# timdestan/go-raytracer

Measured on AMD Instinct MI355X. Metric: Mrays/s (primary+shadow+reflect) at 4K depth=6; 1/2/4/8-GPU scaling, higher is better.
Workload: dtype f64; 1 GPU; c3: cylinder + cube + sphere (cone substitute) over a reflective plane, 4 lights, 3840x2160, depth 6; width=3840, height=2160, depth=6, lights=4, objects=4, parallelism=rows1-interleaved, frames_in_flight=2, schedule=auto, kernel=specialised, accel=bvh+cull

## Files before the change

go-raytracer_amd/csrc/rt_kernel.hip:

```cpp
#pragma clang fp contract(off)

#include <hip/hip_runtime.h>

#include <dlfcn.h>
#include <errno.h>
#include <fcntl.h>
#include <hip/hiprtc.h>
#include <sys/syscall.h>
#include <sys/wait.h>
#include <unistd.h>

#include <algorithm>
#include <atomic>
#include <chrono>
#include <condition_variable>
#include <cstdlib>
#include <functional>
#include <thread>
#include <cmath>
#include <array>
#include <cstdio>
#include <utility>
#include <cstring>
#include <limits>
// ... 466 lines not shown
  uint64_t* gboard = nullptr;
  uint64_t* gring = nullptr;
  uint64_t* gctl = nullptr;
  size_t gslots = 0;
  int gframes = 0;
  unsigned int* est = nullptr;
  size_t est_cap = 0;
  unsigned long long* est_stats = nullptr;
  std::vector<uint32_t> tile_cost;
  double order_ms = 0;
  std::map<std::array<int, 5>, unsigned int*> orders;
  bool specialize = false;
  int accel = RT_ACCEL_BVH | RT_ACCEL_CULL;
  hipFunction_t spec_fn = nullptr;
  std::map<int, hipFunction_t> spec_alt;
  SpecKey spec_key;
  double spec_ms = 0;
  bool spec_async = false;
  bool spec_fallback = false;
  bool spec_pending = false;
  bool spec_failed = false;
  std::string spec_err;
  bool last_spec = false;
};

namespace {

struct DeviceGuard {
  int prev = -1;
  explicit DeviceGuard(int dev) {
    if (hipGetDevice(&prev) != hipSuccess) prev = -1;
    if (prev != dev) (void)hipSetDevice(dev);
  }
  ~DeviceGuard() {
    if (prev >= 0) (void)hipSetDevice(prev);
  }
};

void free_scene(DevScene& s) {
  (void)hipFree(s.blob);
  (void)hipFree(s.accel);
  s = DevScene();
}

void clear_orders(rt_context* c) {
  for (auto& kv : c->orders) (void)hipFree(kv.second);
// ... 1443 lines not shown
  {
    const int top = n / topd;
    const int tail = taild > 0 ? std::min(n - top, n / taild) : 0;
    std::vector<char> cls(n, 1);
    for (int i = 0; i < top; i++) cls[ord[i]] = 0;
    for (int i = n - tail; i < n; i++) cls[ord[i]] = 2;
    int k = top;
    for (int v = 0; v < n; v++)
      if (cls[v] == 1) ord[k++] = (uint32_t)v;
    for (int v = 0; v < n; v++)
      if (cls[v] == 2) ord[k++] = (uint32_t)v;
  }
  unsigned int* d = nullptr;
  HIP_TRY(hipMalloc((void**)&d, (size_t)n * sizeof(unsigned int)));
  if (hipMemcpy(d, ord.data(), (size_t)n * sizeof(unsigned int), hipMemcpyHostToDevice) != hipSuccess) {
    (void)hipFree(d);
    return fail(RT_E_DEVICE, "tile order upload failed");
  }
  c->orders[key] = d;
  *out = d;
  return RT_OK;
}

static int launch(rt_context* c, int y0, int y1, int trow0, int stride, int ntrows, void* d_rgba, void* stream,
                  bool est) {
  const DevScene& s = c->sc;
  DeviceGuard guard(c->device);
  hipStream_t st = (hipStream_t)stream;
  if (c->spec_pending && !est) (void)spec_prepare(c);
  const bool lds = scene_in_lds(s);
  const int vm_off = lds ? s.blob_bytes : 0;
  const int stack_off = vm_off + ((lds && s.num_programs) ? WG * MAT * (int)sizeof(double) : 0);
  const int cnt_off = stack_off + (s.use_bvh ? WAVES_PER_WG * BVH_STACK * 12 : 0);
  const int qmask_off = cnt_off + CNT_BYTES;
  const int jump_off = qmask_off + 16;
  const int board_off = jump_off + 20 * 4 * (int)sizeof(uint64_t);
  const uint64_t launch_pixels = (uint64_t)s.width * (uint64_t)(stride > 0 ? ntrows * TILE : y1 - y0);
  const int sch =
      est ? (int)SCH_SERIAL : pick_schedule(c->sched, s, launch_pixels, c->cus, c->inflight, c->spec_fn != nullptr);
  const int share_m = (c->spec_fn && !est) ? pick_share(c->share_mode, s, launch_pixels, c->cus, c->inflight) : 0;
  hipFunction_t spec = nullptr;
  if (!est) {
    int rc = spec_for(c, sch, share_m, &spec);
    if (rc != RT_OK) return rc;
  }
  static const bool spec_extra = rt_getenv("RT_SPEC_EXTRA_FLAGS") != nullptr;
  const bool use_stream = !lds && !s.use_bvh && !s.has_csg && (spec_extra || !(spec && !(c->accel & RT_ACCEL_CULL)));
  const bool quads = sch == SCH_QUADS || (sch == SCH_PAIRS && !spec);
  const void* kfn = k_kernels[kernel_index(lds, s.use_bvh, s.has_csg, quads, s.ext_code)];
  const bool share = spec && share_m == RT_SHARE_GROUP;
  const int stream_off = board_off + (share ? BOARD_BYTES : 0);
  const int frames_off = stream_off + (use_stream ? WAVES_PER_WG * SCH * (GEO * (int)sizeof(double) + (int)sizeof(int)) : 0);
  int shmem = frames_off;
  auto occupancy = [&](int bytes) {
    int n = 0;
    if (spec) {
      if (hipModuleOccupancyMaxActiveBlocksPerMultiprocessor(&n, spec, WG, bytes) != hipSuccess) n = 0;
    } else if (hipOccupancyMaxActiveBlocksPerMultiprocessor(&n, kfn, WG, bytes) != hipSuccess) {
      n = 0;
    }
    return n;
  };
  const void* plan_fn = spec ? (const void*)spec : kfn;
  const int frames = std::max(1, s.depth - 1);
  LaunchPlan& pl = c->plan;
  const bool plan_hit = pl.fn == plan_fn && pl.shmem_fixed == shmem && pl.frames == frames;
  int per_cu = plan_hit ? pl.per_cu : occupancy(shmem);
  if (per_cu <= 0) per_cu = 1;
  const int level_bytes = WAVES_PER_WG * CORE * 64 * (int)sizeof(double);
  const int ext_bytes = WAVES_PER_WG * EXT_ROWS * 64 * (int)sizeof(double);
  int lds_levels = plan_hit ? pl.lds_levels : 0, lds_full = plan_hit ? pl.lds_full : 0;
  if (!plan_hit && c->lds_per_cu > 0 && c->lds_per_block > 0) {
    const int avail = std::min(c->lds_per_block, c->lds_per_cu / std::min(per_cu, 8)) - shmem;
    if (const char* e = rt_getenv("RT_LDS_FULL")) lds_full = std::max(0, std::min(frames, atoi(e)));
    while (lds_full > 0 && lds_full * (ext_bytes + level_bytes) > avail) lds_full--;
    lds_levels = std::max(lds_full, std::min(frames, (avail - lds_full * ext_bytes) / level_bytes));
    if (const char* e = rt_getenv("RT_LDS_LEVELS")) lds_levels = std::max(lds_full, std::min(lds_levels, atoi(e)));
    while (lds_levels > 0 && occupancy(shmem + lds_levels * level_bytes + lds_full * ext_bytes) < per_cu) {
      lds_levels--;
      lds_full = std::min(lds_full, lds_levels);
    }
  }
  if (!plan_hit) pl = LaunchPlan{plan_fn, shmem, frames, per_cu, lds_levels, lds_full};
  const int ext_off = shmem + lds_levels * level_bytes;
  shmem = ext_off + lds_full * ext_bytes;
  static const bool dbg = rt_getenv("RT_DEBUG_LAUNCH") != nullptr;
  if (dbg)
    fprintf(stderr, "[launch] blocks/CU %d, LDS/block %d B (fixed %d, frame cores %d levels, full frames %d levels), frames %d\n",
            per_cu, shmem, frames_off, lds_levels, lds_full, frames);
  const int grid = c->cus * std::min(per_cu, 8);
  c->last_waves = grid * WAVES_PER_WG;
  c->launches++;
  if (grid * WAVES_PER_WG > c->stack_waves) return fail(RT_E_INVALID, "frame stack smaller than the grid");
  if (spec && share_m == RT_SHARE_DEVICE) {
    const size_t need = (size_t)c->stack_waves * 64 * frames;
    if (need != c->gslots || frames != c->gframes) {
      (void)hipFree(c->gboard);
      c->gboard = nullptr;
      c->gslots = 0;
      if (hipExtMallocWithFlags((void**)&c->gboard, need * GS_REC * sizeof(uint64_t), hipDeviceMallocUncached) !=
          hipSuccess)
        return fail(RT_E_NOMEM, "device-wide work-sharing slots");
      if (!c->gring && hipExtMallocWithFlags((void**)&c->gring, (size_t)GS_RING * sizeof(uint64_t),
                                             hipDeviceMallocUncached) != hipSuccess)
        return fail(RT_E_NOMEM, "device-wide work-sharing ring");
      if (!c->gctl && hipExtMallocWithFlags((void**)&c->gctl, GS_CTL_U64 * sizeof(uint64_t), hipDeviceMallocUncached) !=
                          hipSuccess)
        return fail(RT_E_NOMEM, "device-wide work-sharing control");
      HIP_TRY(hipMemsetAsync(c->gboard, 0, need * GS_REC * sizeof(uint64_t), st));
      HIP_TRY(hipMemsetAsync(c->gring, 0, (size_t)GS_RING * sizeof(uint64_t), st));
      HIP_TRY(hipMemsetAsync(c->gctl, 0, GS_CTL_U64 * sizeof(uint64_t), st));
      c->gslots = need;
      c->gframes = frames;
    }
  }
  Params P;
  std::memset(&P, 0, sizeof P);
  P.lds_frames_off = frames_off;
  P.lds_levels = lds_levels;
  P.lds_full = lds_full;
  P.stream_off = stream_off;
  P.lds_ext_off = ext_off;
  P.qmask_off = qmask_off;
  P.jump_off = jump_off;
  P.board_off = board_off;
  P.gboard = c->gboard;
  P.gring = c->gring;
  P.gctl = c->gctl;
  P.gslots = c->gslots;
  P.gset = c->qset;
  P.off_geo = s.off_geo;
  P.off_shade = s.off_shade;
  P.off_mats = s.off_mats;
  P.off_lights = s.off_lights;
  P.off_kind = s.off_kind;
  P.off_objmat = s.off_objmat;
  P.off_pref = s.off_prefb;
  P.off_csg = s.off_csg;
  P.off_code = s.off_code;
  P.off_consts = s.off_consts;
  P.off_entry = s.off_entry;
  P.lds_vm_off = vm_off;
  P.vm_global = c->vm_global;
  P.blob_bytes = s.blob_bytes;
  P.jump = c->jump;
  P.queue = c->queue + c->qset * QSET_ALLOC;
  P.queue_next = c->queue + (1 - c->qset) * QSET_ALLOC;
  P.stats = est ? c->est_stats : c->stats;
// ... 112 lines not shown
  c->order_ms = std::chrono::duration<double, std::milli>(std::chrono::steady_clock::now() - t0).count();
  c->timed = false;
  return RT_OK;
}

int rt_set_work_sharing(rt_context* c, int enable) {
  if (!c) return fail(RT_E_INVALID, "rt_set_work_sharing: NULL context");
  if (enable < 0 || enable > RT_SHARE_AUTO) return fail(RT_E_INVALID, "rt_set_work_sharing: unknown mode");
  c->share_mode = enable;
  return c->has_scene ? spec_prepare(c) : RT_OK;
}

int rt_set_tile_order(rt_context* c, int enable) {
  if (!c) return fail(RT_E_INVALID, "rt_set_tile_order: NULL context");
  c->order_on = enable != 0;
  if (!c->has_scene) return RT_OK;
  if (!c->order_on) {
    clear_orders(c);
    return RT_OK;
  }
  return c->tile_cost.empty() ? estimate_costs(c) : RT_OK;
}

int rt_tile_order_info(rt_context* c, int* active, double* estimate_ms) {
  if (!c || !active || !estimate_ms) return fail(RT_E_INVALID, "rt_tile_order_info: NULL argument");
  *active = c->tile_cost.empty() ? 0 : 1;
  *estimate_ms = c->order_ms;
  return RT_OK;
}

int rt_render_rows_async(rt_context* c, int y0, int y1, void* d_rgba, void* stream) {
  if (!c || !c->has_scene) return fail(RT_E_INVALID, "rt_render_rows_async: no scene set");
  if (!d_rgba) return fail(RT_E_INVALID, "rt_render_rows_async: NULL output");
  if (y0 < 0 || y1 > c->sc.height || y1 <= y0) return fail(RT_E_INVALID, "rt_render_rows_async: bad row range");
  return launch(c, y0, y1, 0, 0, 0, d_rgba, stream, false);
}

int rt_render_tile_rows_async(rt_context* c, int trow0, int trow_stride, int ntrows, void* d_rgba, void* stream) {
  if (!c || !c->has_scene) return fail(RT_E_INVALID, "rt_render_tile_rows_async: no scene set");
  if (!d_rgba) return fail(RT_E_INVALID, "rt_render_tile_rows_async: NULL output");
  if (trow0 < 0 || trow_stride <= 0 || ntrows <= 0) return fail(RT_E_INVALID, "rt_render_tile_rows_async: bad tile rows");
  return launch(c, 0, c->sc.height, trow0, trow_stride, ntrows, d_rgba, stream, false);
}


int rt_read_stats(rt_context* c, void* stream, int reset, rt_stats* out) {
// ... 182 lines not shown
```

go-raytracer_amd/csrc/rt_render.h:

```cpp
#pragma once
#pragma clang fp contract(off)

#ifndef __HIPCC_RTC__
#include <hip/hip_runtime.h>
#endif

#include "rt_abi.h"
#include "rt_device.h"

#ifndef RT_SHADE_NUM
#define RT_SHADE_NUM 3
#endif
#ifndef RT_SHADE_DEN
#define RT_SHADE_DEN 4
#endif
#ifndef RT_DIV_SKIP
#define RT_DIV_SKIP 0
#endif
#ifndef RT_PIX_BATCH
#define RT_PIX_BATCH 1
#endif
#ifndef RT_PAIRS
#define RT_PAIRS 0
#endif
// ... 121 lines not shown
  int trow0, trow_stride;
  unsigned int total_slots;
  int frames;
  const float* bvh_nodes;
  const double* bvh_geo;
  const int* planes;
  int nplanes, bvh_stack_off;
  double bvh_lo[3], bvh_hi[3];
  const int* runs;
  int nruns;
  const double* arec;
  const double* urec;
  int cnt_off;
  int kind_mask;
  int board_off;
  uint64_t* gboard;
  uint64_t* gring;
  uint64_t* gctl;
  int gset;
  unsigned long long gslots;
  const unsigned int* order;
  unsigned int* est_out;
  int est_pts;
};
enum { CNT_TRACED = 0, CNT_SHADED = 1, CNT_SURFERR = 2, NUNIT = 3, CNT_KIND_OFF = 128,
       CNT_BYTES = CNT_KIND_OFF + RT_NUM_KINDS * WG * 8 };
enum { PREF = 8 };
enum { BN = 16, BVH_STACK = 64 };

struct Ray {
  d3 o, d;
};

template <typename MP>
__device__ __forceinline__ d3 to_obj_o(MP m, d3 o) {
  return mk(m[0] * o.x + m[1] * o.y + m[2] * o.z + m[3], m[4] * o.x + m[5] * o.y + m[6] * o.z + m[7],
            m[8] * o.x + m[9] * o.y + m[10] * o.z + m[11]);
}
template <typename MP>
__device__ __forceinline__ d3 to_obj_d(MP m, d3 d) {
  return mk(m[0] * d.x + m[1] * d.y + m[2] * d.z, m[4] * d.x + m[5] * d.y + m[6] * d.z,
            m[8] * d.x + m[9] * d.y + m[10] * d.z);
}
template <typename MP>
__device__ __forceinline__ Ray to_obj(MP m, const Ray& r) {
  Ray l;
  l.o = to_obj_o(m, r.o);
// ... 1417 lines not shown
    }
  };
  const d3 eye = mk(0.0, 0.0, -1.0);

  int state = S_IDLE;
  bool need_gen = false;
  int px = 0, py = 0, sample = 0, sp = 0;
  unsigned int pout = 0;
  uint32_t held_px = ~0u, held_val = 0u;
  auto flush_pixels = [&]() {
    if (held_px != ~0u) P.out[held_px] = held_val;
    held_px = ~0u;
  };
#ifndef RT_WAVE_SGPR
#define RT_WAVE_SGPR (BVH || CSG)
#endif
  const int wave = RT_WAVE_SGPR ? __builtin_amdgcn_readfirstlane((int)(threadIdx.x >> 6)) : (int)(threadIdx.x >> 6);
  int my_idle = 0, spins = 0;
  bool my_active = true;
  bool sh_live = false;
  int hit_i = 0, hit_f = 0;
  double hit_t = 0.0;
  Pcg rng{0, 0};
  d3 sum = mk(0, 0, 0);
  d3 sum2 = mk(0, 0, 0);
  Ray ray;
  ray.o = mk(0, 0, 0);
  ray.d = mk(0, 0, 1);

  unsigned int pool_next = 0, pool_end = 0;
  int qhead = 0;
  bool exhausted = false;
  unsigned long long* cnt = reinterpret_cast<unsigned long long*>(smem + P.cnt_off);
  unsigned long long* kcnt = reinterpret_cast<unsigned long long*>(smem + P.cnt_off + CNT_KIND_OFF);
  for (int k = 0; k < RT_NUM_KINDS; k++) kcnt[k * WG + threadIdx.x] = 0;
#ifndef RT_CNT_REMAT
#define RT_CNT_REMAT (BVH || CSG)
#endif
  auto opaque_s = [](uint32_t b) {
    b = (uint32_t)__builtin_amdgcn_readfirstlane((int)b);
    asm volatile("" : "+s"(b));
    return b;
  };
  auto cnt_kind = [&](int k, uint64_t v) {
    if constexpr (RT_CNT_REMAT) {
      uint32_t l;
      asm volatile("v_mbcnt_lo_u32_b32 %0, -1, 0\n\tv_mbcnt_hi_u32_b32 %0, -1, %0" : "=v"(l));
      const uint32_t a = opaque_s((uint32_t)P.cnt_off + (uint32_t)(CNT_KIND_OFF + (k * WG + wave * 64) * 8)) + l * 8u;
// ... 29 lines not shown
  const double W1 = (double)(P.width - 1), H1 = (double)(P.height - 1);

  auto gen_ray = [&]() {
    double dx = pcg_float64(rng) - 0.5;
    double dy = pcg_float64(rng) - 0.5;
    const double vw = G[9], vh = G[10];
    double u = ((double)px + dx) / W1 * vw - vw / 2.0;
    double v = ((double)py + dy) / H1 * vh - vh / 2.0;
    ray.o = mk(u, -v, 0.0);
    ray.d = norm(sub(ray.o, eye));
  };

  auto sample_rng = [&](int x, int y, int k) {
    const int ry = y % 20;
    const uint64_t* j = P.jump + (ry * 4 + k) * 4;
    return pcg_jump(Pcg{0xDEADULL ^ (uint64_t)x, 0xBEEFULL ^ (uint64_t)(y - ry)}, j[0], j[1], j[2], j[3]);
  };
  auto wait_slot = [&]() -> int {
    if (RT_SHARE == 1 && !QD && sp == 0) return lw_fork(Bd->lw[threadIdx.x], sample);
    return PK_SLOT_OF(__double_as_longlong(core_ld(sp - 1, 4)));
  };
  auto advance_sample = [&](uint32_t w) {
    for (;;) {
      if (P.est_out && sample == 1) {
        state = S_IDLE;
        return;
      }
      if (PR && sample == ((lane & 1) ? 4 : 2)) {
        state = S_DONE;
        return;
      }
      if (sample == 4) {
        d3 c = scale(sum, 1.0 / 4.0);
        uint32_t r8 = go_f64_to_u32(c.x * 65535.0) >> 8;
        uint32_t g8 = go_f64_to_u32(c.y * 65535.0) >> 8;
        uint32_t b8 = go_f64_to_u32(c.z * 65535.0) >> 8;
#ifdef RT_COST_MAP
        P.out[pout] = lane_cost;
        lane_cost = 0;
#else
        const uint32_t v = (r8 & 0xffu) | ((g8 & 0xffu) << 8) | ((b8 & 0xffu) << 16) | 0xff000000u;
        if (RT_PIX_BATCH) {
          held_px = pout;
          held_val = v;
        } else {
          P.out[pout] = v;
        }
// ... 133 lines not shown
    if (++guard_iters > (1u << 26)) {
      if (lane == 0) atomicAdd(P.stats + ST_WATCHDOG, 1ull);
      break;
    }
    if constexpr (!QD) {
      if (wave_any(state == S_ADV)) {
        if (RT_PIX_BATCH && wave_any(state == S_ADV && held_px != ~0u && (RT_SHARE || (!PR && sample == 4)))) flush_pixels();
        if (state == S_ADV) {
          const uint32_t w = RT_SHARE == 1 ? Bd->lw[threadIdx.x] : 4u;
          if (RT_SHARE == 1 && __builtin_expect(lw_task(w) >= 0, 0)) {
            board_deliver(Bd, lw_task(w), sum);
            Bd->lw[threadIdx.x] = 0u;
            state = S_IDLE;
          } else {
            advance_sample(w);
          }
        }
      }
    }
    if constexpr (QD) {
      const uint64_t dn = wave_ballot(state == S_DONE);
      const uint64_t qd = dn & (dn >> 1) & (dn >> 2) & (dn >> 3) & 0x1111111111111111ull;
      if (qd) {
        d3 sm = add(mk(0, 0, 0), sum);
#pragma unroll
        for (int k = 1; k < 4; k++) {
          const int lk = (lane + k) & 63;
          sm = add(sm, mk(__shfl(sum.x, lk), __shfl(sum.y, lk), __shfl(sum.z, lk)));
        }
        if (RT_PIX_BATCH && wave_any(((qd >> lane) & 1) && held_px != ~0u)) flush_pixels();
        if ((qd >> lane) & 1) {
          const d3 c = scale(sm, 1.0 / 4.0);
          const uint32_t r8 = go_f64_to_u32(c.x * 65535.0) >> 8;
          const uint32_t g8 = go_f64_to_u32(c.y * 65535.0) >> 8;
          const uint32_t b8 = go_f64_to_u32(c.z * 65535.0) >> 8;
          const uint32_t v = (r8 & 0xffu) | ((g8 & 0xffu) << 8) | ((b8 & 0xffu) << 16) | 0xff000000u;
          if (RT_PIX_BATCH) {
            held_px = pout;
            held_val = v;
          } else {
            P.out[pout] = v;
          }
        }
        if ((qd >> (lane & ~3)) & 1) state = S_IDLE;
      }
    }
    if constexpr (PR) {
      const uint64_t dn = wave_ballot(state == S_DONE);
      const uint64_t pd = dn & (dn >> 1) & 0x5555555555555555ull;
      if (pd) {
        const int lb = (lane + 1) & 63;
        const d3 c2 = mk(__shfl(sum.x, lb), __shfl(sum.y, lb), __shfl(sum.z, lb));
        const d3 c3 = mk(__shfl(sum2.x, lb), __shfl(sum2.y, lb), __shfl(sum2.z, lb));
        const d3 sm = add(add(sum, c2), c3);
        if (RT_PIX_BATCH && wave_any(((pd >> lane) & 1) && held_px != ~0u)) flush_pixels();
        if ((pd >> lane) & 1) {
          const d3 c = scale(sm, 1.0 / 4.0);
          const uint32_t r8 = go_f64_to_u32(c.x * 65535.0) >> 8;
          const uint32_t g8 = go_f64_to_u32(c.y * 65535.0) >> 8;
          const uint32_t b8 = go_f64_to_u32(c.z * 65535.0) >> 8;
          const uint32_t v = (r8 & 0xffu) | ((g8 & 0xffu) << 8) | ((b8 & 0xffu) << 16) | 0xff000000u;
          if (RT_PIX_BATCH) {
            held_px = pout;
            held_val = v;
          } else {
            P.out[pout] = v;
          }
        }
        if ((pd >> (lane & ~1)) & 1) state = S_IDLE;
      }
    }
    for (;;) {
      const uint64_t il = wave_ballot(state == S_IDLE);
      const uint64_t mask = QD   ? il & (il >> 1) & (il >> 2) & (il >> 3) & 0x1111111111111111ull
                            : PR ? il & (il >> 1) & 0x5555555555555555ull
                                 : il;
      const bool need = ((mask >> (QD ? (lane & ~3) : PR ? (lane & ~1) : lane)) & 1) != 0;
// ... 12 lines not shown
          unsigned int n = 0;
          if (lane == 0) n = atomicAdd(P.queue + h * QSTRIDE, 1u);
          c = __builtin_amdgcn_readfirstlane(n) * QHEADS + h;
          if (c < nchunks) break;
          if (lane == 0) atomicOr(qdrained, 1u << h);
          qhead++;
        }
        if (qhead >= nheads) {
          exhausted = true;
          break;
        }
#ifdef RT_PHASE_TIMING
        last_grab = stamp();
        nchunk_taken++;
#endif
        pool_next = c * QCHUNK;
        pool_end = min(pool_next + (unsigned int)QCHUNK, P.total_slots);
      }
      const unsigned int rank = QD   ? (unsigned int)__popcll(mask & ((1ull << (lane & ~3)) - 1ull))
                                : PR ? (unsigned int)__popcll(mask & ((1ull << (lane & ~1)) - 1ull))
                                     : __builtin_amdgcn_mbcnt_hi((unsigned int)(mask >> 32),
                                                                 __builtin_amdgcn_mbcnt_lo((unsigned int)mask, 0u));
      unsigned int take = min((unsigned int)__popcll(mask), pool_end - pool_next);
      if (!QD && !PR && P.est_out) {
        if (need && rank < take) {
          const unsigned int u = pool_next + rank, t = u / (unsigned)P.est_pts, k = u % (unsigned)P.est_pts;
          px = min((int)(t % (unsigned)P.tiles_x) * TILE + est_x(P.est_pts, k), P.width - 1);
          py = min((int)(t / (unsigned)P.tiles_x) * TILE + est_y(P.est_pts, k), P.y1 - 1);
          pout = t;
          const int ry = py % 20;
          rng = pcg_jump(Pcg{0xDEADULL ^ (uint64_t)px, 0xBEEFULL ^ (uint64_t)(py - ry)}, jrows[ry * 4],
                         jrows[ry * 4 + 1], jrows[ry * 4 + 2], jrows[ry * 4 + 3]);
          sample = 0;
          if (RT_SHARE == 1) Bd->lw[threadIdx.x] = 1u;
          sum = mk(0, 0, 0);
          sp = 0;
          need_gen = true;
          state = S_TRACE;
        }
        pool_next += take;
        continue;
      }
      unsigned int tile = pool_next / (TILE * TILE);
      if (P.order) tile = P.order[tile];
      const int trow = (int)(tile / (unsigned)P.tiles_x);
      const int x0 = (int)((tile % (unsigned)P.tiles_x) * TILE);
      const int orow0 = trow * TILE;
// ... 88 lines not shown
            gs_st(r + 3, (uint64_t)__double_as_longlong(dd.x));
            gs_st(r + 4, (uint64_t)__double_as_longlong(dd.y));
            gs_st(r + 5, (uint64_t)__double_as_longlong(dd.z));
            gs_st(r + 6, (uint64_t)(L + 1));
            gs_drain();
            gs_st(r + 7, GS_POSTED);
            const long long pk = __double_as_longlong(core_ld(L, 4));
            core_st(L, 4, __longlong_as_double(pk | FL_FORKED | ((long long)q << PK_SLOT)));
          }
          gs_drain();
          uint64_t t0 = 0;
          if (lane == 0) t0 = __hip_atomic_fetch_add(g_tail, (uint64_t)npost, __ATOMIC_RELAXED, RT_AG_SCOPE);
          t0 = rfl64(t0);
          if (post) {
            const uint64_t t = t0 + (uint64_t)rk;
            gs_st(g_ring + (t & (GS_RSH - 1)), (t << 32) | (uint32_t)q);
          }
        }
      }
      uint64_t il = exhausted ? wave_ballot(state == S_IDLE) : 0ull;
      int cshard = gshard;
      uint64_t ch = gh;
      bool ctry = outstanding > 0;
      if (GS_SH > 1 && il != 0 && !ctry && gs_helper && (guard_iters & 3u) == 0u && !P.est_out) {
        const int k = lane < GS_SH ? (gshard + 1 + lane) % GS_SH : gshard;
        uint64_t ot = 0, oh = 0;
        if (lane < GS_SH - 1) {
          ot = gs_ld(P.gctl + GS_SHARD * k + GS_TAIL);
          oh = gs_ld(P.gctl + GS_SHARD * k + GS_HEAD);
        }
        const uint64_t hasm = wave_ballot(lane < GS_SH - 1 && ot > oh);
        if (hasm) {
          const int fl = __builtin_ctzll(hasm);
          cshard = (gshard + 1 + fl) % GS_SH;
          ch = rfl64(__shfl(oh, fl));
          ctry = true;
        }
      }
      if (__builtin_expect(il != 0 && ctry && !P.est_out, 0)) {
        uint64_t* const c_head = P.gctl + GS_SHARD * cshard + GS_HEAD;
        uint64_t* const c_tail = P.gctl + GS_SHARD * cshard + GS_TAIL;
        uint64_t* const c_ring = P.gring + (size_t)cshard * GS_RSH;
        const int nil = (int)__popcll(il);
        uint64_t h = 0;
        int k = 0;
        if (lane == 0) {
          uint64_t hh = ch;
          for (int tries = 0; tries < 4; tries++) {
            const uint64_t tt = gs_ld(c_tail);
            const int kk = tt > hh ? (int)min((uint64_t)nil, tt - hh) : 0;
            if (kk <= 0) break;
            if (__hip_atomic_compare_exchange_strong(c_head, &hh, hh + (uint64_t)kk, __ATOMIC_RELAXED,
                                                     __ATOMIC_RELAXED, RT_AG_SCOPE)) {
              h = hh;
              k = kk;
              break;
            }
          }
        }
        h = rfl64(h);
        k = __builtin_amdgcn_readfirstlane(k);
        if (k > 0) {
// ... 6 lines not shown
              e = gs_ld(c_ring + (t & (GS_RSH - 1)));
              if ((uint32_t)(e >> 32) == (uint32_t)t) break;
              __builtin_amdgcn_s_sleep(1);
            }
            if ((uint32_t)(e >> 32) == (uint32_t)t && (uint32_t)e < P.gslots) {
              const int q = (int)(uint32_t)e;
              uint64_t* r = gs_slot(P.gboard, q);
              if (gs_claim(r)) {
                SHDIAG(SH_CLAIM);
                ray.o = mk(__longlong_as_double((long long)gs_ld(r + 0)), __longlong_as_double((long long)gs_ld(r + 1)),
                           __longlong_as_double((long long)gs_ld(r + 2)));
                ray.d = mk(__longlong_as_double((long long)gs_ld(r + 3)), __longlong_as_double((long long)gs_ld(r + 4)),
                           __longlong_as_double((long long)gs_ld(r + 5)));
                const int m0 = (int)gs_ld(r + 6);
                core_st(m0 - 1, 4, __longlong_as_double((long long)FL_TASK | ((long long)q << PK_SLOT)));
                sp = m0;
                state = S_TRACE;
              }
            }
          }
          il = wave_ballot(state == S_IDLE);
        }
      }
      const int cur_idle = (exhausted && !P.est_out) ? (int)__popcll(il) : 0;
      if (cur_idle != my_idle) {
        nidle_add(cur_idle - my_idle);
        my_idle = cur_idle;
      }
      const bool busy = wave_any(state != S_IDLE);
      if (busy != my_active) {
        if (lane == 0) atomicAdd(g_active, busy ? 1u : 0xffffffffu);
        my_active = busy;
      }
      if (__builtin_expect(!busy, 0)) {
        if (!gs_helper) {
          unsigned int old = 0;
          if (lane == 0) old = atomicAdd(g_helpers, 1u);
          gs_helper = __builtin_amdgcn_readfirstlane((int)old) < RT_GS_HELPERS;
          if (!gs_helper) {
            if (my_idle) nidle_add(-my_idle);
            break;
          }
        }
        const int na = (spins & 7) ? 1 : __builtin_amdgcn_readfirstlane(lane == 0 ? (int)gs_ld32(g_active) : 0);
        if (na == 0 || ++spins > RT_SHARE_SPINS) {
#ifdef RT_PHASE_TIMING
          if (lane == 0) atomicAdd(P.stats + ST_SHDIAG + SH_SPIN, (unsigned long long)spins);
// ... 89 lines not shown
            SHDIAG(SH_CLAIM);
            const int m0 = Bd->meta[q][0];
            if (m0 & META_SAMPLE) {
              px = m0 & 0xffff;
              py = Bd->meta[q][1];
              sample = (m0 >> 16) & 3;
              Bd->lw[threadIdx.x] = (uint32_t)(sample + 1) | ((uint32_t)(q + 1) << 3);
              sum = mk(-0.0, -0.0, -0.0);
              rng = sample_rng(px, py, sample);
              need_gen = true;
              sp = 0;
            } else {
              ray.o = mk(Bd->ray[q][0], Bd->ray[q][1], Bd->ray[q][2]);
              ray.d = mk(Bd->ray[q][3], Bd->ray[q][4], Bd->ray[q][5]);
              core_st(m0 - 1, 4, __longlong_as_double((long long)FL_TASK | ((long long)q << PK_SLOT)));
              Bd->lw[threadIdx.x] = 0u;
              sp = m0;
            }
            state = S_TRACE;
          }
          il = wave_ballot(state == S_IDLE);
        }
      }
      const int cur_idle = P.est_out ? 0 : (int)__popcll(il);
      if (cur_idle != my_idle) {
        if (lane == 0) __hip_atomic_fetch_add(&Bd->nidle, cur_idle - my_idle, __ATOMIC_RELAXED, RT_WG_SCOPE);
        my_idle = cur_idle;
      }
      const bool busy = wave_any(state != S_IDLE);
      if (busy != my_active) {
        if (lane == 0) __hip_atomic_fetch_add(&Bd->nactive, busy ? 1 : -1, __ATOMIC_RELAXED, RT_WG_SCOPE);
        my_active = busy;
      }
      if (__builtin_expect(!busy, 0)) {
        const int na = __builtin_amdgcn_readfirstlane(__hip_atomic_load(&Bd->nactive, __ATOMIC_RELAXED, RT_WG_SCOPE));
        const uint64_t pm = __hip_atomic_load(&Bd->post, __ATOMIC_RELAXED, RT_WG_SCOPE);
        if ((na == 0 && __builtin_amdgcn_readfirstlane((int)(pm >> 32)) == 0 &&
             __builtin_amdgcn_readfirstlane((int)pm) == 0) ||
            ++spins > RT_SHARE_SPINS) {
#ifdef RT_PHASE_TIMING
          if (lane == 0) atomicAdd(P.stats + ST_SHDIAG + SH_SPIN, (unsigned long long)spins);
#endif
          if (lane == 0 && my_idle) __hip_atomic_fetch_add(&Bd->nidle, -my_idle, __ATOMIC_RELAXED, RT_WG_SCOPE);
          break;
        }
        __builtin_amdgcn_s_sleep(RT_SHARE_SLEEP);
        continue;
// ... 252 lines not shown
            const bool a0 = may_hit_box_a(act, bof, idf, bslack, tmax, nb, t0);
            const bool a1 = may_hit_box_a(act, bof, idf, bslack, tmax, nb + 6, t1);
            const uint64_t m0 = wave_ballot(a0), m1 = wave_ballot(a1);
            const bool c1_first = 2 * __popcll(wave_ballot(a0 && a1 && t1 < t0)) > __popcll(m0 & m1);
#if RT_BVH_CONT
            bvh_next(bst, ssp, lane, c1_first, ni[0], ni[1], m0, m1, nr, nm, have);
#else
            if (c1_first) {
              if (m0) bst.push(ssp, lane, ni[0], m0);
              if (m1) bst.push(ssp, lane, ni[1], m1);
            } else {
              if (m1) bst.push(ssp, lane, ni[1], m1);
              if (m0) bst.push(ssp, lane, ni[0], m0);
            }
#endif
          }
        }
      }
      cnt_unit(CNT_TRACED, tr);
#ifdef RT_PHASE_TIMING
      pd_tr++;
      pd_trl += (uint64_t)__popcll(wave_ballot(tr));
#endif
      if (!QD && P.est_out && tr) atomicAdd(P.est_out + pout, 1u);
      PH_MARK(2);
      d3 res = mk(0, 0, 0);
      if (tr) {
        if (found) {
          state = S_SHADE;
          hit_i = best_i;
          hit_f = best_f;
          hit_t = best_t;
        } else {
          double t = 0.5 * (ray.d.y + 1.0);
          res = lerp(mk(G[3], G[4], G[5]), mk(G[6], G[7], G[8]), t);
        }
      }
      const bool resumed = RT_SHARE && state == S_RESUME;
      if (__builtin_expect(resumed, 0))
        res = RT_SHARE == 2 ? gs_take(P.gboard, wait_slot()) : board_take(Bd, wait_slot());
      unwind((tr && !found) || resumed, res, pf, pf_packed, pf_lw, pf_kr);
      PH_MARK(3);
    }

    const uint64_t nsh = popc_ballot(state == S_SHADE);
    const uint64_t ntr = popc_ballot(state == S_TRACE ||
                                     (!QD && state == S_ADV && (RT_SHARE || sample < (PR && !(lane & 1) ? 2 : 4))));
// ... 71 lines not shown
        }
        vmrec[7] = r[5];
        vmrec[8] = r[6];
        vmrec[9] = r[7];
        vmrec[10] = r[8];
        vmrec[11] = r[9];
        vmrec[12] = 1.0 / vmrec[8];
        const double r0 = (1.0 - vmrec[8]) / (1.0 + vmrec[8]);
        vmrec[13] = r0 * r0;
        surf_bad = bad;
      }
    }
    cnt_unit(CNT_SURFERR, surf_bad);

    PH_MARK(4);
    const double* M = (!spec_feat(SF_VM) || mat >= 0) ? S.mats + (size_t)mat * MAT : vmrec;
    d3 L = mk(0, 0, 0);
    if (hit) L = scale(mk(G[0], G[1], G[2]), M[9]);
    const double rlen = len(ray.d);
#if RT_STMAX_F32
    const float rlen_rcpf = __builtin_amdgcn_rcpf((float)rlen);
#endif
    const d3 sorig = add(pw, scale(nw, 1e-4));
#define SH_PLANE_CULL(i, d, tmax) may_hit_plane(sof, d, tmax, SHP(i))
    uint32_t sc0 = 0, sc1 = 0, sc2 = 0, sc3 = 0;
    auto light_dir = [&](auto lt, d3& ldir, double& dist) {
      if (spec_feat(SF_LDIR) && (int)lt[9] == RT_LIGHT_DIRECTIONAL) {
        ldir = mk(lt[6], lt[7], lt[8]);
        dist = __builtin_inf();
      } else {
        d3 lth = sub(mk(lt[0], lt[1], lt[2]), pw);
        ldir = norm_len(lth, dist);
      }
    };
#ifdef RT_SPEC_NLIGHTS
    d3 ldir_a[RT_SPEC_NLIGHTS];
    double dist_a[RT_SPEC_NLIGHTS];
#pragma unroll
    for (int li = 0; li < RT_SPEC_NLIGHTS; li++) light_dir(LTP(li), ldir_a[li], dist_a[li]);
    PH_MARK(5);
#if RT_STREAM_SMEM && !RT_CULL && RT_SHADOW_JOINT && !defined(RT_SPEC_NOBJ) && RT_SPEC_NLIGHTS <= 4
#define RT_JOINT_SWEEP 1
#else
#define RT_JOINT_SWEEP 0
#endif
#if RT_JOINT_SWEEP
    bool jopen[RT_SPEC_NLIGHTS];
// ... 552 lines not shown
```

go-raytracer_amd/render.py:

```python
import ctypes as C
import os

import numpy as np

from . import abi
from . import scene as _scene

PKG_DIR = os.path.dirname(os.path.abspath(__file__))
LIB_PATH = os.path.join(PKG_DIR, "csrc", "librtamd.so")

_lib = None


class RenderError(RuntimeError):
    pass


def load_library(path=None):
    global _lib
    if _lib is not None:
        return _lib
    path = path or os.environ.get("RT_AMD_LIB") or LIB_PATH
    if not os.path.exists(path):
        raise RenderError("HIP renderer library not built: %s (run __graft_entry__.build())" % path)
# ... 34 lines not shown
    l.rt_specialized.restype = i
    l.rt_spec_precompile.argtypes = [i, C.POINTER(i), i, C.POINTER(C.c_double)]
    l.rt_spec_precompile.restype = i
    l.rt_set_work_sharing.argtypes = [vp, i]
    l.rt_set_work_sharing.restype = i
    l.rt_set_tile_order.argtypes = [vp, i]
    l.rt_set_tile_order.restype = i
    l.rt_set_frames_in_flight.argtypes = [vp, i]
    l.rt_set_frames_in_flight.restype = i
    l.rt_tile_order_info.argtypes = [vp, C.POINTER(i), C.POINTER(C.c_double)]
    l.rt_tile_order_info.restype = i
    l.rt_render.argtypes = [vp, vp, vp]
    l.rt_render.restype = i
    l.rt_render_last_timing.argtypes = [vp]
    l.rt_render_last_timing.restype = i
    l.rt_render_ex.argtypes = [vp, vp, vp, vp]
    l.rt_render_ex.restype = i
    l.rt_debug_assemble.argtypes = [i, i, i, i, vp, vp]
    l.rt_debug_assemble.restype = i
    l.rt_debug_spec_compile.argtypes = [C.c_char_p, C.POINTER(C.c_double)]
    l.rt_debug_spec_compile.restype = i
    l.rt_debug_getenv.argtypes = [C.c_char_p]
    l.rt_debug_getenv.restype = C.c_char_p
    l.rt_query_closest_async.argtypes = [vp, i, vp, vp, vp]
    l.rt_query_closest_async.restype = i
    l.rt_query_occluded_async.argtypes = [vp, i, vp, vp, vp]
    l.rt_query_occluded_async.restype = i
    if l.rt_abi_version() != abi.RT_ABI_VERSION:
        raise RenderError("librtamd ABI version mismatch")
    _lib = l
    return l


def _check(rc, what):
    if rc != abi.RT_OK:
        msg = _lib.rt_last_error() if _lib is not None else b""
        raise RenderError("%s failed (%d): %s" % (what, rc, (msg or b"").decode(errors="replace")))


def _packed(scene_or_args):
    if isinstance(scene_or_args, abi.PackedScene):
        return scene_or_args
    return _scene.convert(scene_or_args)


class RenderContext:

    def __init__(self, device=None, specialize=False):
        import torch
        if not torch.cuda.is_available():
            raise RenderError("no HIP device visible: the renderer has no CPU path")
        self.torch = torch
        self.lib = load_library()
        self.device = torch.cuda.current_device() if device is None else int(device)
# ... 29 lines not shown

    def set_schedule(self, mode):
        _check(self.lib.rt_set_schedule(self.handle, int(mode)), "rt_set_schedule")

    def set_tile_order(self, enable=True):
        _check(self.lib.rt_set_tile_order(self.handle, int(bool(enable))), "rt_set_tile_order")

    def set_frames_in_flight(self, n):
        _check(self.lib.rt_set_frames_in_flight(self.handle, int(n)), "rt_set_frames_in_flight")

    def set_work_sharing(self, enable=True):
        mode = int(enable)
        _check(self.lib.rt_set_work_sharing(self.handle, mode), "rt_set_work_sharing")

    def tile_order_info(self):
        a, ms = C.c_int(), C.c_double()
        _check(self.lib.rt_tile_order_info(self.handle, C.byref(a), C.byref(ms)), "rt_tile_order_info")
        return bool(a.value), ms.value

    def scene_info(self):
        f = C.c_int()
        _check(self.lib.rt_scene_info(self.handle, C.byref(f)), "rt_scene_info")
        return f.value

    def specialized(self):
        a, ms = C.c_int(), C.c_double()
        _check(self.lib.rt_specialized(self.handle, C.byref(a), C.byref(ms)), "rt_specialized")
        return bool(a.value), ms.value

    def render_rows_async(self, y0, y1, out, stream=None):
        torch = self.torch
        W = self.packed.width
        assert out.dtype == torch.uint8 and out.is_cuda and out.is_contiguous()
        assert out.numel() == (y1 - y0) * W * 4, "output tensor shape does not match rows"
        s = torch.cuda.current_stream(self.device) if stream is None else stream
        _check(self.lib.rt_render_rows_async(self.handle, int(y0), int(y1), C.c_void_p(out.data_ptr()),
                                             C.c_void_p(s.cuda_stream)), "rt_render_rows_async")

    def render_tile_rows_async(self, trow0, stride, ntrows, out, stream=None):
        torch = self.torch
        W = self.packed.width
        assert out.dtype == torch.uint8 and out.is_cuda and out.is_contiguous()
        assert out.numel() == ntrows * 8 * W * 4, "output tensor shape does not match tile rows"
        s = torch.cuda.current_stream(self.device) if stream is None else stream
        _check(self.lib.rt_render_tile_rows_async(self.handle, int(trow0), int(stride), int(ntrows),
                                                  C.c_void_p(out.data_ptr()), C.c_void_p(s.cuda_stream)),
# ... 190 lines not shown
```

include/rt_abi.h:

```cpp
#ifndef RT_ABI_H
#define RT_ABI_H

#ifndef __HIPCC_RTC__
#include <stddef.h>
#endif
#include <stdint.h>

#ifdef __cplusplus
extern "C" {
#endif

#define RT_ABI_VERSION 6
#define RT_MAX_DEVICES 16
#define RT_EXP_AMD64_FMA 0
#define RT_EXP_AMD64 1
#define RT_EXP_PORTABLE 2

#define RT_OK 0
#define RT_E_INVALID (-1)
#define RT_E_SINGULAR (-2)
#define RT_E_DEVICE (-3)
#define RT_E_NOMEM (-4)

#define RT_SPHERE 0
// ... 154 lines not shown

int rt_set_specialize(rt_context *ctx, int enable);

#define RT_ACCEL_BVH 1
#define RT_ACCEL_CULL 2
int rt_set_accel(rt_context *ctx, int flags);

#define RT_SCHED_AUTO 0
#define RT_SCHED_PIXEL 1
#define RT_SCHED_QUADS 2
#define RT_SCHED_PAIRS 3
int rt_set_schedule(rt_context *ctx, int mode);

int rt_set_frames_in_flight(rt_context *ctx, int n);

int rt_set_tile_order(rt_context *ctx, int enable);
#define RT_SHARE_OFF 0
#define RT_SHARE_GROUP 1
#define RT_SHARE_DEVICE 2
#define RT_SHARE_AUTO 3
int rt_set_work_sharing(rt_context *ctx, int enable);
int rt_tile_order_info(rt_context *ctx, int *active, double *estimate_ms);

#define RT_INFO_LDS 1
#define RT_INFO_BVH 2
#define RT_INFO_CSG 4
#define RT_INFO_STREAM 8
#define RT_INFO_WAVEFRONT 16
#define RT_INFO_ORDERED 32
#define RT_INFO_SHARE_DEVICE 64
int rt_scene_info(rt_context *ctx, int *flags);

int rt_specialized(rt_context *ctx, int *active, double *compile_ms);

#define RT_SPEC_SURFACES 1
#define RT_SPEC_DIRECTIONAL 2
#define RT_SPEC_SPOT 4
#define RT_SPEC_LIGHTS(n) ((n) << 8)
int rt_spec_precompile(int nobj, const int *kinds, int features, double *compile_ms);

int rt_debug_spec_compile(const char *key, double *compile_ms);

const char *rt_debug_getenv(const char *name);

int rt_debug_run_surface(rt_context *ctx, int program, int n, const long long *face,
                         const double *u, const double *v, double *out10, int *err);
// ... 70 lines not shown
```

Baseline: 73200 Mrays/s.

## Park per-pixel accumulators in LDS and hoist shadow plane culling in specialised kernels

```diff
diff --git a/go-raytracer_amd/csrc/rt_kernel.hip b/go-raytracer_amd/csrc/rt_kernel.hip
--- a/go-raytracer_amd/csrc/rt_kernel.hip
+++ b/go-raytracer_amd/csrc/rt_kernel.hip
@@ -512,6 +512,7 @@
   bool spec_failed = false;
   std::string spec_err;
   bool last_spec = false;
+  std::array<int, 5> last_lds{{0, 0, 0, 0, 0}};
 };
 
 namespace {
@@ -2001,6 +2002,24 @@
   return RT_OK;
 }
 
+struct LdsLayout {
+  int vm_off, stack_off, cnt_off, qmask_off, jump_off, board_off, park_off, stream_off, frames_off;
+};
+static LdsLayout lds_layout(int blob_lds_bytes, bool vm_records, bool bvh, bool board, int park, bool stream) {
+  LdsLayout l;
+  l.vm_off = blob_lds_bytes;
+  l.stack_off = l.vm_off + (vm_records ? WG * MAT * (int)sizeof(double) : 0);
+  l.cnt_off = l.stack_off + (bvh ? WAVES_PER_WG * BVH_STACK * 12 : 0);
+  l.qmask_off = l.cnt_off + CNT_BYTES;
+  l.jump_off = l.qmask_off + 16;
+  l.board_off = l.jump_off + 20 * 4 * (int)sizeof(uint64_t);
+  l.park_off = l.board_off + (board ? BOARD_BYTES : 0);
+  l.stream_off = l.park_off + park;
+  l.frames_off = l.stream_off + (stream ? WAVES_PER_WG * SCH * (GEO * (int)sizeof(double) + (int)sizeof(int)) : 0);
+  return l;
+}
+static_assert(BOARD_BYTES % 16 == 0 && CNT_BYTES % 16 == 0, "LDS sections stay 16-byte aligned");
+
 static int launch(rt_context* c, int y0, int y1, int trow0, int stride, int ntrows, void* d_rgba, void* stream,
                   bool est) {
   const DevScene& s = c->sc;
@@ -2008,12 +2027,6 @@
   hipStream_t st = (hipStream_t)stream;
   if (c->spec_pending && !est) (void)spec_prepare(c);
   const bool lds = scene_in_lds(s);
-  const int vm_off = lds ? s.blob_bytes : 0;
-  const int stack_off = vm_off + ((lds && s.num_programs) ? WG * MAT * (int)sizeof(double) : 0);
-  const int cnt_off = stack_off + (s.use_bvh ? WAVES_PER_WG * BVH_STACK * 12 : 0);
-  const int qmask_off = cnt_off + CNT_BYTES;
-  const int jump_off = qmask_off + 16;
-  const int board_off = jump_off + 20 * 4 * (int)sizeof(uint64_t);
   const uint64_t launch_pixels = (uint64_t)s.width * (uint64_t)(stride > 0 ? ntrows * TILE : y1 - y0);
   const int sch =
       est ? (int)SCH_SERIAL : pick_schedule(c->sched, s, launch_pixels, c->cus, c->inflight, c->spec_fn != nullptr);
@@ -2028,8 +2041,10 @@
   const bool quads = sch == SCH_QUADS || (sch == SCH_PAIRS && !spec);
   const void* kfn = k_kernels[kernel_index(lds, s.use_bvh, s.has_csg, quads, s.ext_code)];
   const bool share = spec && share_m == RT_SHARE_GROUP;
-  const int stream_off = board_off + (share ? BOARD_BYTES : 0);
-  const int frames_off = stream_off + (use_stream ? WAVES_PER_WG * SCH * (GEO * (int)sizeof(double) + (int)sizeof(int)) : 0);
+  const int park = (spec && c->spec_key.nobj > 0) ? park_bytes(sch == SCH_PAIRS) : 0;
+  const LdsLayout lay = lds_layout(lds ? s.blob_bytes : 0, lds && s.num_programs, s.use_bvh, share, park, use_stream);
+  const int vm_off = lay.vm_off, stack_off = lay.stack_off, cnt_off = lay.cnt_off, qmask_off = lay.qmask_off,
+            jump_off = lay.jump_off, board_off = lay.board_off, stream_off = lay.stream_off, frames_off = lay.frames_off;
   int shmem = frames_off;
   auto occupancy = [&](int bytes) {
     int n = 0;
@@ -2050,7 +2065,8 @@
   const int ext_bytes = WAVES_PER_WG * EXT_ROWS * 64 * (int)sizeof(double);
   int lds_levels = plan_hit ? pl.lds_levels : 0, lds_full = plan_hit ? pl.lds_full : 0;
   if (!plan_hit && c->lds_per_cu > 0 && c->lds_per_block > 0) {
-    const int avail = std::min(c->lds_per_block, c->lds_per_cu / std::min(per_cu, 8)) - shmem;
+    const int granule = 1280;
+    const int avail = std::min(c->lds_per_block, c->lds_per_cu / std::min(per_cu, 8) / granule * granule) - shmem;
     if (const char* e = rt_getenv("RT_LDS_FULL")) lds_full = std::max(0, std::min(frames, atoi(e)));
     while (lds_full > 0 && lds_full * (ext_bytes + level_bytes) > avail) lds_full--;
     lds_levels = std::max(lds_full, std::min(frames, (avail - lds_full * ext_bytes) / level_bytes));
@@ -2068,6 +2084,7 @@
     fprintf(stderr, "[launch] blocks/CU %d, LDS/block %d B (fixed %d, frame cores %d levels, full frames %d levels), frames %d\n",
             per_cu, shmem, frames_off, lds_levels, lds_full, frames);
   const int grid = c->cus * std::min(per_cu, 8);
+  c->last_lds = {frames_off, lay.park_off, park, shmem, per_cu};
   c->last_waves = grid * WAVES_PER_WG;
   c->launches++;
   if (grid * WAVES_PER_WG > c->stack_waves) return fail(RT_E_INVALID, "frame stack smaller than the grid");
@@ -2103,6 +2120,7 @@
   P.qmask_off = qmask_off;
   P.jump_off = jump_off;
   P.board_off = board_off;
+  P.park_off = lay.park_off;
   P.gboard = c->gboard;
   P.gring = c->gring;
   P.gctl = c->gctl;
@@ -2261,6 +2279,34 @@
   return c->tile_cost.empty() ? estimate_costs(c) : RT_OK;
 }
 
+int rt_debug_launch_lds(rt_context* c, int out[5]) {
+  if (!c || !out) return fail(RT_E_INVALID, "rt_debug_launch_lds: NULL argument");
+  if (!c->last_lds[0]) return fail(RT_E_INVALID, "rt_debug_launch_lds: nothing launched yet");
+  for (int k = 0; k < 5; k++) out[k] = c->last_lds[k];
+  return RT_OK;
+}
+
+int rt_debug_lds_layout(int nobj, int nmats, int nlights, int schedule, int specialised, int out[4]) {
+  if (!out || nobj < 1 || nmats < 0 || nlights < 0) return fail(RT_E_INVALID, "rt_debug_lds_layout: bad argument");
+  if (schedule != RT_SCHED_PIXEL && schedule != RT_SCHED_QUADS && schedule != RT_SCHED_PAIRS)
+    return fail(RT_E_INVALID, "rt_debug_lds_layout: schedule must be pixel, quads or pairs");
+  int b = align16(nobj * GEO * (int)sizeof(double));
+  b = align16(b + nobj * SHD * (int)sizeof(double));
+  b = align16(b + nmats * MAT * (int)sizeof(double));
+  b = align16(b + (GLOB + std::max(1, nlights) * LGT) * (int)sizeof(double));
+  b = align16(b + nobj * (int)sizeof(int));
+  b = align16(b + nobj * OMAT * (int)sizeof(int));
+  b = align16(b + (nobj + 1) * PREF * (int)sizeof(uint32_t));
+  const bool parks = specialised && nobj <= SPEC_MAX_OBJ;
+  const int park = parks ? park_bytes(schedule == RT_SCHED_PAIRS) : 0;
+  const LdsLayout l = lds_layout(b <= (int)LDS_MAX_BYTES ? b : 0, false, false, false, park, false);
+  out[0] = l.frames_off;
+  out[1] = l.park_off;
+  out[2] = park;
+  out[3] = b;
+  return RT_OK;
+}
+
 int rt_tile_order_info(rt_context* c, int* active, double* estimate_ms) {
   if (!c || !active || !estimate_ms) return fail(RT_E_INVALID, "rt_tile_order_info: NULL argument");
   *active = c->tile_cost.empty() ? 0 : 1;
diff --git a/go-raytracer_amd/csrc/rt_render.h b/go-raytracer_amd/csrc/rt_render.h
--- a/go-raytracer_amd/csrc/rt_render.h
+++ b/go-raytracer_amd/csrc/rt_render.h
@@ -167,7 +167,33 @@
   const unsigned int* order;
   unsigned int* est_out;
   int est_pts;
+  int park_off;
 };
+#ifndef RT_PARK
+#ifdef RT_SPEC_NOBJ
+#define RT_PARK 1
+#else
+#define RT_PARK 0
+#endif
+#endif
+#if RT_PARK && !defined(RT_SPEC_NOBJ)
+#error "RT_PARK: the host lays out the parked state only for the specialised small-scene kernels"
+#endif
+__host__ __device__ constexpr int park_bytes(bool pairs) { return (pairs ? 6 : 3) * WG * (int)sizeof(double); }
+struct ParkedD3 {
+  double* p;
+  __device__ __forceinline__ operator d3() const { return mk(p[0], p[WG], p[2 * WG]); }
+  __device__ __forceinline__ void operator=(const d3& v) {
+    p[0] = v.x;
+    p[WG] = v.y;
+    p[2 * WG] = v.z;
+  }
+};
+#ifdef RT_SPEC_NOBJ
+#define EST_OUT ((unsigned int*)nullptr)
+#else
+#define EST_OUT P.est_out
+#endif
 enum { CNT_TRACED = 0, CNT_SHADED = 1, CNT_SURFERR = 2, NUNIT = 3, CNT_KIND_OFF = 128,
        CNT_BYTES = CNT_KIND_OFF + RT_NUM_KINDS * WG * 8 };
 enum { PREF = 8 };
@@ -1631,8 +1657,13 @@
   int hit_i = 0, hit_f = 0;
   double hit_t = 0.0;
   Pcg rng{0, 0};
+#if RT_PARK
+  double* const park = reinterpret_cast<double*>(smem + P.park_off) + threadIdx.x;
+  ParkedD3 sum{park}, sum2{park + 3 * WG};
+#else
   d3 sum = mk(0, 0, 0);
   d3 sum2 = mk(0, 0, 0);
+#endif
   Ray ray;
   ray.o = mk(0, 0, 0);
   ray.d = mk(0, 0, 1);
@@ -1708,7 +1739,7 @@
   };
   auto advance_sample = [&](uint32_t w) {
     for (;;) {
-      if (P.est_out && sample == 1) {
+      if (EST_OUT && sample == 1) {
         state = S_IDLE;
         return;
       }
@@ -1888,11 +1919,12 @@
       const uint64_t dn = wave_ballot(state == S_DONE);
       const uint64_t qd = dn & (dn >> 1) & (dn >> 2) & (dn >> 3) & 0x1111111111111111ull;
       if (qd) {
-        d3 sm = add(mk(0, 0, 0), sum);
+        const d3& own = sum;
+        d3 sm = add(mk(0, 0, 0), own);
 #pragma unroll
         for (int k = 1; k < 4; k++) {
           const int lk = (lane + k) & 63;
-          sm = add(sm, mk(__shfl(sum.x, lk), __shfl(sum.y, lk), __shfl(sum.z, lk)));
+          sm = add(sm, mk(__shfl(own.x, lk), __shfl(own.y, lk), __shfl(own.z, lk)));
         }
         if (RT_PIX_BATCH && wave_any(((qd >> lane) & 1) && held_px != ~0u)) flush_pixels();
         if ((qd >> lane) & 1) {
@@ -1916,9 +1948,10 @@
       const uint64_t pd = dn & (dn >> 1) & 0x5555555555555555ull;
       if (pd) {
         const int lb = (lane + 1) & 63;
-        const d3 c2 = mk(__shfl(sum.x, lb), __shfl(sum.y, lb), __shfl(sum.z, lb));
-        const d3 c3 = mk(__shfl(sum2.x, lb), __shfl(sum2.y, lb), __shfl(sum2.z, lb));
-        const d3 sm = add(add(sum, c2), c3);
+        const d3 &own = sum, &own2 = sum2;
+        const d3 c2 = mk(__shfl(own.x, lb), __shfl(own.y, lb), __shfl(own.z, lb));
+        const d3 c3 = mk(__shfl(own2.x, lb), __shfl(own2.y, lb), __shfl(own2.z, lb));
+        const d3 sm = add(add(own, c2), c3);
         if (RT_PIX_BATCH && wave_any(((pd >> lane) & 1) && held_px != ~0u)) flush_pixels();
         if ((pd >> lane) & 1) {
           const d3 c = scale(sm, 1.0 / 4.0);
@@ -1977,7 +2010,7 @@
                                      : __builtin_amdgcn_mbcnt_hi((unsigned int)(mask >> 32),
                                                                  __builtin_amdgcn_mbcnt_lo((unsigned int)mask, 0u));
       unsigned int take = min((unsigned int)__popcll(mask), pool_end - pool_next);
-      if (!QD && !PR && P.est_out) {
+      if (!QD && !PR && EST_OUT) {
         if (need && rank < take) {
           const unsigned int u = pool_next + rank, t = u / (unsigned)P.est_pts, k = u % (unsigned)P.est_pts;
           px = min((int)(t % (unsigned)P.tiles_x) * TILE + est_x(P.est_pts, k), P.width - 1);
@@ -2112,7 +2145,7 @@
       int cshard = gshard;
       uint64_t ch = gh;
       bool ctry = outstanding > 0;
-      if (GS_SH > 1 && il != 0 && !ctry && gs_helper && (guard_iters & 3u) == 0u && !P.est_out) {
+      if (GS_SH > 1 && il != 0 && !ctry && gs_helper && (guard_iters & 3u) == 0u && !EST_OUT) {
         const int k = lane < GS_SH ? (gshard + 1 + lane) % GS_SH : gshard;
         uint64_t ot = 0, oh = 0;
         if (lane < GS_SH - 1) {
@@ -2127,7 +2160,7 @@
           ctry = true;
         }
       }
-      if (__builtin_expect(il != 0 && ctry && !P.est_out, 0)) {
+      if (__builtin_expect(il != 0 && ctry && !EST_OUT, 0)) {
         uint64_t* const c_head = P.gctl + GS_SHARD * cshard + GS_HEAD;
         uint64_t* const c_tail = P.gctl + GS_SHARD * cshard + GS_TAIL;
         uint64_t* const c_ring = P.gring + (size_t)cshard * GS_RSH;
@@ -2180,7 +2213,7 @@
           il = wave_ballot(state == S_IDLE);
         }
       }
-      const int cur_idle = (exhausted && !P.est_out) ? (int)__popcll(il) : 0;
+      const int cur_idle = (exhausted && !EST_OUT) ? (int)__popcll(il) : 0;
       if (cur_idle != my_idle) {
         nidle_add(cur_idle - my_idle);
         my_idle = cur_idle;
@@ -2316,7 +2349,7 @@
           il = wave_ballot(state == S_IDLE);
         }
       }
-      const int cur_idle = P.est_out ? 0 : (int)__popcll(il);
+      const int cur_idle = EST_OUT ? 0 : (int)__popcll(il);
       if (cur_idle != my_idle) {
         if (lane == 0) __hip_atomic_fetch_add(&Bd->nidle, cur_idle - my_idle, __ATOMIC_RELAXED, RT_WG_SCOPE);
         my_idle = cur_idle;
@@ -2615,7 +2648,7 @@
       pd_tr++;
       pd_trl += (uint64_t)__popcll(wave_ballot(tr));
 #endif
-      if (!QD && P.est_out && tr) atomicAdd(P.est_out + pout, 1u);
+      if (!QD && EST_OUT && tr) atomicAdd(EST_OUT + pout, 1u);
       PH_MARK(2);
       d3 res = mk(0, 0, 0);
       if (tr) {
@@ -2733,7 +2766,25 @@
     const float rlen_rcpf = __builtin_amdgcn_rcpf((float)rlen);
 #endif
     const d3 sorig = add(pw, scale(nw, 1e-4));
+#ifndef RT_HOIST_PLANE
+#if defined(RT_SPEC_NOBJ) && defined(RT_SPEC_NLIGHTS) && RT_CULL && RT_PARK
+#define RT_HOIST_PLANE 1
+#else
+#define RT_HOIST_PLANE 0
+#endif
+#endif
+#if RT_HOIST_PLANE
+    PlaneO h_po[RT_SPEC_NOBJ];
+    {
+      const F3 hsof = f3(sorig);
+#pragma unroll
+      for (int i = 0; i < RT_SPEC_NOBJ; i++)
+        if (spec_kinds[i] == RT_PLANE) h_po[i] = may_hit_plane_o(hsof, SHP(i));
+    }
+#define SH_PLANE_CULL(i, d, tmax) may_hit_plane_d(h_po[i], d, tmax, SHP(i))
+#else
 #define SH_PLANE_CULL(i, d, tmax) may_hit_plane(sof, d, tmax, SHP(i))
+#endif
     uint32_t sc0 = 0, sc1 = 0, sc2 = 0, sc3 = 0;
     auto light_dir = [&](auto lt, d3& ldir, double& dist) {
       if (spec_feat(SF_LDIR) && (int)lt[9] == RT_LIGHT_DIRECTIONAL) {
diff --git a/go-raytracer_amd/render.py b/go-raytracer_amd/render.py
--- a/go-raytracer_amd/render.py
+++ b/go-raytracer_amd/render.py
@@ -80,6 +80,10 @@
     l.rt_debug_spec_compile.restype = i
     l.rt_debug_getenv.argtypes = [C.c_char_p]
     l.rt_debug_getenv.restype = C.c_char_p
+    l.rt_debug_launch_lds.argtypes = [vp, C.POINTER(i * 5)]
+    l.rt_debug_launch_lds.restype = i
+    l.rt_debug_lds_layout.argtypes = [i, i, i, i, i, C.POINTER(i * 4)]
+    l.rt_debug_lds_layout.restype = i
     l.rt_query_closest_async.argtypes = [vp, i, vp, vp, vp]
     l.rt_query_closest_async.restype = i
     l.rt_query_occluded_async.argtypes = [vp, i, vp, vp, vp]
@@ -88,6 +92,14 @@
         raise RenderError("librtamd ABI version mismatch")
     _lib = l
     return l
+
+
+def lds_layout(nobj, nmats, nlights, schedule, specialised):
+    l = load_library()
+    o = (C.c_int * 4)()
+    _check(l.rt_debug_lds_layout(int(nobj), int(nmats), int(nlights), int(schedule), int(bool(specialised)),
+                                 C.byref(o)), "rt_debug_lds_layout")
+    return dict(zip(("fixed", "park_off", "park_bytes", "blob_bytes"), list(o)))
 
 
 def _check(rc, what):
@@ -163,6 +175,11 @@
         f = C.c_int()
         _check(self.lib.rt_scene_info(self.handle, C.byref(f)), "rt_scene_info")
         return f.value
+
+    def launch_lds(self):
+        o = (C.c_int * 5)()
+        _check(self.lib.rt_debug_launch_lds(self.handle, C.byref(o)), "rt_debug_launch_lds")
+        return dict(zip(("fixed", "park_off", "park_bytes", "total", "per_cu"), list(o)))
 
     def specialized(self):
         a, ms = C.c_int(), C.c_double()
diff --git a/include/rt_abi.h b/include/rt_abi.h
--- a/include/rt_abi.h
+++ b/include/rt_abi.h
@@ -200,6 +200,10 @@
 int rt_set_work_sharing(rt_context *ctx, int enable);
 int rt_tile_order_info(rt_context *ctx, int *active, double *estimate_ms);
 
+int rt_debug_launch_lds(rt_context *ctx, int out[5]);
+
+int rt_debug_lds_layout(int nobj, int nmats, int nlights, int schedule, int specialised, int out[4]);
+
 #define RT_INFO_LDS 1
 #define RT_INFO_BVH 2
 #define RT_INFO_CSG 4
```

Result: no change. 73730 Mrays/s, median of 6 (+0.7%).
